# rsokolovskii/fl_scaling_sc_ldpc

Hardware: AMD Instinct MI355X
Metric: MC codeword trials/sec, (4,8) SC-LDPC L=50 N=1000 eps=0.48 full BP (higher is better)
Workload: dtype u32

## Files before the change

### fl_scaling_sc_ldpc_amd/csrc/full_bp_small.hip

```cpp
#include "common.h"
#include "kernel_util.h"
#include "table_rows.h"
#include <algorithm>
#include <cstdlib>
#include <type_traits>

namespace {

using namespace scldpc_dev;

enum { SC_NE = 0, SC_REM, SC_N0, SC_N1, SC_OVF, SC_Q, SC_N = 8 };
enum { LV_VALID = 2, LV_EXTRA0 = 3, LV_PUSH = 6, LV_DROP = 9, LV_REM = 12, LV_OVF = 15, LV_N = 18 };

struct SmArgs {
    int L, V, C, n, nk, cn_lim, nw, ncw;
    uint32_t magic_v, magic_c;
    int ntrials;
    int kswitch;
    int max_it;
    int rows_cap;
    int32_t *rows;
    int off_U, off_q0, off_q1, off_pos, off_scal, off_fb, total, qcap;
    const uint16_t *vn_adj16;
    const uint16_t *cn_adj16;
    const uint32_t *chan;
    int32_t *counters;
    uint32_t *erased_out;
    int ncaps;
    int caps[SCLDPC_MAX_CAPS];
};


template <int BLOCK, bool LEVEL, bool PERSIST, bool SOCK, bool TRAJ = false, bool CAPS = false, bool WIDE = false, int DV = 4, int DC = 8,
          int OCC = 0>
__global__ __launch_bounds__(BLOCK, OCC ? OCC : WIDE ? 4 : PERSIST ? 8 : 7) __attribute__((amdgpu_num_sgpr(96))) void full_bp_small_kernel(const SmArgs a)
{
    static_assert(!WIDE || (BLOCK == 1024 && LEVEL && SOCK && !PERSIST), "the wide form: LEVEL [+ TRAJ | CAPS], socket table");
    static_assert(!(TRAJ && CAPS), "the checkpoints have no rows form");
    static_assert((DV == 4 && DC == 8) || (SOCK && !PERSIST), "other degree pairs: the socket table, no PERSIST");
    static_assert(DC <= 15 && DC % 2 == 0 && DV < DC, "a CN's count of erased neighbours is a nibble; CN rows are read as 32-bit words");
    using QT = std::conditional_t<WIDE, uint32_t, uint16_t>;
    constexpr int kWaves = BLOCK / 64;
    extern __shared__ uint32_t lds[];
    uint32_t *cnt = lds;
    uint32_t *U = lds + a.off_U;
    QT *q[2] = {reinterpret_cast<QT *>(lds + a.off_q0), reinterpret_cast<QT *>(lds + a.off_q1)};
    int *pos_cnt = reinterpret_cast<int *>(lds + a.off_pos);
    int *pos_ss = pos_cnt + a.L;
    int *scal = reinterpret_cast<int *>(lds + a.off_scal);

    const int tid = threadIdx.x, lane = tid & 63, wave = tid >> 6;
    auto decode_trial = [&](const int trial) {
    STAMP_DECL
    const int n = a.n, nk = a.nk, cn_lim = a.cn_lim, nw = a.nw, V = a.V, C = a.C, L = a.L, qcap = a.qcap;
    const auto *vrow = reinterpret_cast<const typename VnUnit<DV>::type *>(a.vn_adj16) + (size_t)trial * n * VnUnit<DV>::per_row;
    const auto *crow = reinterpret_cast<const typename CnUnit<DC>::type *>(a.cn_adj16) + (size_t)trial * nk * CnUnit<DC>::per_row;
    auto vn_row = [&](int j) { if constexpr (DV == 4) return load_row(vrow, j); else return load_row<DV>(vrow, j); };
    auto cn_row = [&](int c) { if constexpr (DC == 8) return load_row(crow, c); else return load_row<DC>(crow, c); };
    const uint32_t *ch = a.chan + (size_t)trial * nw;

    for (int c = tid; c < a.ncw; c += BLOCK) cnt[c] = 0;
    int ne_local = 0;
    for (int w = tid; w < nw; w += BLOCK) {
        const uint32_t x = chan_tail(ch[w], w, nw, n);
        U[w] = x;
        ne_local += __popc(x);
    }
    if (tid < LV_N) scal[tid] = 0;
    for (int i = tid; i < 2 * L; i += BLOCK) pos_cnt[i] = 0;
    __syncthreads();
    ne_local = wave_sum(ne_local);
    if (lane == 0 && ne_local) atomicAdd(&scal[SC_NE], ne_local);

    constexpr int NB = 8;
    for (int j0 = tid; j0 < n; j0 += NB * BLOCK) {
        Row<DV> r[NB];
        bool er[NB];
#pragma unroll
        for (int u = 0; u < NB; u++) {
            const int j = j0 + u * BLOCK;
            er[u] = false;
            if (j < n) { r[u] = vn_row(j); er[u] = (U[j >> 5] >> (j & 31)) & 1u; }
        }
#pragma unroll
        for (int u = 0; u < NB; u++) {
            const int j = j0 + u * BLOCK;
            if (er[u]) {
                const int base = (int)__umulhi((uint32_t)j, a.magic_v) * C;
                int cc[DV];
#pragma unroll
                for (int i = 0; i < DV; i++) cc[i] = base + i * C + (int)r[u][i];
#pragma unroll
                for (int i = 0; i < DV; i++) atomicAdd(&cnt[cc[i] >> 3], 1u << ((cc[i] & 7) * 4));
            }
        }
    }
    __syncthreads();
    STAMP(0);
    const int nch = scal[SC_NE];

    int removed = 0, drops = 0;
    auto step = [&](int c, uint32_t (&out)[DV]) {
#pragma unroll
        for (int i = 0; i < DV; i++) out[i] = 0;
        const Row<DC> s = cn_row(c);
        uint32_t jk[DC];
        bool none[DC];
#pragma unroll
        for (int k = 0; k < DC; k++) { jk[k] = s[k]; none[k] = jk[k] == 0xFFFFu; }
        if constexpr (SOCK) {
            const int vbase = (int)__umulhi((uint32_t)c, a.magic_c) * V;
#pragma unroll
            for (int k = 0; k < DC; k++) jk[k] = (uint32_t)(vbase - (int)(jk[k] % DV) * V) + (jk[k] / DV);
        }
        uint32_t wd[DC];
#pragma unroll
        for (int k = 0; k < DC; k++) wd[k] = U[none[k] ? 0u : jk[k] >> 5];
        int j = -1;
#pragma unroll
        for (int k = 0; k < DC; k++)
            if (!none[k] && ((wd[k] >> (jk[k] & 31u)) & 1u)) j = (int)jk[k];
        if (j < 0) return;
        const Row<DV> r = vn_row(j);
        const uint32_t bit = 1u << (j & 31);
        if (!(atomicAnd(&U[j >> 5], ~bit) & bit)) return;
        removed++;
        const int base = (int)__umulhi((uint32_t)j, a.magic_v) * C;
        int cc[DV];
#pragma unroll
        for (int i = 0; i < DV; i++) cc[i] = base + i * C + (int)r[i];
        uint32_t o[DV];
#pragma unroll
        for (int i = 0; i < DV; i++) o[i] = atomicSub(&cnt[cc[i] >> 3], 1u << ((cc[i] & 7) * 4));
#pragma unroll
        for (int i = 0; i < DV; i++) {
            const uint32_t old = (o[i] >> ((cc[i] & 7) * 4)) & 15u;
            if (old == 2u && cc[i] < cn_lim) out[i] = (uint32_t)cc[i] + 1u;
            if constexpr (LEVEL) drops += (old == 1u && cc[i] < cn_lim);
        }
    };
    auto ones_of = [&](int w) {
        const uint32_t y = cnt[w] ^ 0x11111111u;
        uint32_t z = ~(((y & 0x77777777u) + 0x77777777u) | y) & 0x88888888u;
        if (w * 8 + 8 > cn_lim) {
            const int keep = cn_lim - w * 8;
            z = keep <= 0 ? 0u : (z & ((1u << (4 * keep)) - 1u));
        }
        return z;
    };
    auto append = [&](const uint32_t (&out)[DV], int *push, QT *qn, bool &overflow) {
        int mine = 0;
#pragma unroll
        for (int i = 0; i < DV; i++) mine += out[i] != 0u;
        const int incl = (int)wave_inclusive_scan((uint32_t)mine);
        const int tot = __builtin_amdgcn_readlane(incl, 63);
        if (tot) {
            int base = 0;
            if (lane == 0) base = atomicAdd(push, tot);
            int idx = __builtin_amdgcn_readfirstlane(base) + incl - mine;
#pragma unroll
            for (int i = 0; i < DV; i++)
                if (out[i]) { if (idx < qcap) qn[idx] = (QT)(out[i] - 1u); else overflow = true; idx++; }
        }
    };

    int rounds = 0, ne = 0, status = 0, be = 0, ee = 0, bee = 0;
    auto residual = [&]() {
    if (ne > 0) {
        for (int w = tid; w < nw; w += BLOCK) {
            uint32_t x = U[w];
            int p0 = (int)__umulhi((uint32_t)(w * 32), a.magic_v);
            int room = (p0 + 1) * V - w * 32;
            while (x) {
                const uint32_t lo = room >= 32 ? x : (x & ((1u << room) - 1u));
                if (lo) atomicAdd(&pos_cnt[p0], __popc(lo));
                x = room >= 32 ? 0u : (x >> room);
                p0++;
                room = V;
            }
        }
        __syncthreads();
        int q0 = 0;
        for (;;) {
            while (q0 < L && pos_cnt[q0] == 0) q0++;
            if (q0 >= L) break;
            for (int t = tid; t < V; t += BLOCK) {
                const int j = q0 * V + t;
                if (!((U[j >> 5] >> (j & 31)) & 1u)) continue;
                const Row<DV> r = vn_row(j);
                const int base = q0 * C;
                int cc[DV];
#pragma unroll
                for (int i = 0; i < DV; i++) cc[i] = base + i * C + (int)r[i];
                bool pair = true;
#pragma unroll
                for (int i = 0; i < DV; i++) pair = pair && ((cnt[cc[i] >> 3] >> ((cc[i] & 7) * 4)) & 15u) == 2u;
                if (!pair) continue;
                int partner = -1;
                for (int i = 0; i < DV && pair; i++) {
                    const Row<DC> s = cn_row(cc[i]);
                    int other = -1;
                    for (int k = 0; k < DC; k++) {
                        const uint32_t jk = s[k];
                        if (jk == 0xFFFFu) continue;
                        const int j2 = SOCK ? (q0 + i - (int)(jk % DV)) * V + (int)(jk / DV) : (int)jk;
                        if (j2 != j && ((U[j2 >> 5] >> (j2 & 31)) & 1u)) other = j2;
                    }
                    if (other < 0 || (i > 0 && other != partner)) pair = false;
                    partner = other;
                }
                if (pair && (int)__umulhi((uint32_t)partner, a.magic_v) == q0) atomicAdd(&pos_ss[q0], 1);
            }
            __syncthreads();
            const int e = pos_cnt[q0] - pos_ss[q0];
            if (e > 0) { ee = e; bee = 1; break; }
            q0++;
        }
        for (int pos = 0; pos < L; pos++) be += pos_cnt[pos] > 0;
    }
    };
    auto put = [&](int32_t *o, int ne, int be, int ee, int bee, int rounds, int status) {
        o[SCLDPC_C_NUM_ERASURES] = ne;
        o[SCLDPC_C_NUM_BLOCKS_ERR] = be;
        o[SCLDPC_C_NUM_ERASURES_EXP] = ee;
        o[SCLDPC_C_NUM_BLOCKS_ERR_EXP] = bee;
        o[SCLDPC_C_NUM_ERASURES_P1] = 0;
        o[SCLDPC_C_ITERATIONS] = rounds;
        o[SCLDPC_C_STATUS] = status;
        o[SCLDPC_C_CHANNEL_ERASURES] = nch;
    };
    auto cap_counters = [&](int k) { return a.counters + ((size_t)k * a.ntrials + trial) * SCLDPC_NCOUNTERS; };

    int ci = 0;
    if constexpr (LEVEL) {
        uint8_t *fb = reinterpret_cast<uint8_t *>(lds + a.off_fb);
        int prec = n, iter = 0, ncur = 0, nfront = 0, first_word = 0;
        if constexpr (TRAJ) {
            int extra = 0;
            const int head = (DV - 1) * C, tail0 = L * C;
            for (int i = tid; i < 2 * head; i += BLOCK) {
                const int c = i < head ? i : tail0 + (i - head);
                if (c >= cn_lim || c >= nk) continue;
                const Row<DC> s = cn_row(c);
                int deg = 0;
#pragma unroll
                for (int k = 0; k < DC; k++) deg += s[k] != 0xFFFFu;
                extra += deg == 1 && ((cnt[c >> 3] >> ((c & 7) * 4)) & 15u) == 0u;
            }
            extra = wave_sum(extra);
            if (lane == 0 && extra) atomicAdd(&scal[LV_EXTRA0], extra);
        }
        bool scan = true;
        ne = nch;
        for (;;) {
            const int g = iter % 3, gn = (iter + 1) % 3;
            QT *qc = q[iter & 1], *qn = q[(iter + 1) & 1];
            if (tid == 0) { scal[LV_PUSH + gn] = 0; scal[LV_DROP + gn] = 0; scal[LV_REM + gn] = 0; scal[LV_OVF + gn] = 0; }
// ... 593 lines not shown
```

### fl_scaling_sc_ldpc_amd/csrc/sampler_common.h

```cpp
#pragma once
#include "common.h"
#include "kernel_util.h"
#include <algorithm>
#include <cstdlib>

namespace scldpc {

constexpr int kSamplerThreads = 1024;
constexpr int kSamplerWaves = kSamplerThreads / 64;
constexpr int kMaxDoped = 32;
constexpr int kWorkCap = 1024;

}

namespace scldpc_dev {

__device__ __forceinline__ uint32_t channel_erased(uint32_t draw, uint32_t thresh) { return (uint32_t)((draw >> 1) < thresh); }
__device__ __forceinline__ uint32_t channel_tail(uint32_t word, int j0, int n)
{
    if (j0 + 32 > n) word &= (1u << (n - j0)) - 1u;
    return word;
}
__device__ __forceinline__ uint32_t channel_undope(uint32_t word, int j0, int pos, int vns_pos)
{
    const int lo = max(pos * vns_pos, j0) - j0, hi = min((pos + 1) * vns_pos, j0 + 32) - j0;
    if (lo < hi) word &= ~(((hi - lo) == 32 ? 0xFFFFFFFFu : ((1u << (hi - lo)) - 1u)) << lo);
    return word;
}

__device__ __forceinline__ uint32_t nib_sum(uint32_t x)
{
    const uint32_t v = (x & 0x0F0Fu) + ((x >> 4) & 0x0F0Fu);
    return (v + (v >> 8)) & 0xFFu;
}

template <int ROWS>
__device__ __forceinline__ void load_hist_words(const uint32_t *hist, int tid, uint32_t (&x)[ROWS])
{
    if constexpr (ROWS % 4 == 0) {
#pragma unroll
        for (int r = 0; r < ROWS / 4; r++) {
            const uint4 q = reinterpret_cast<const uint4 *>(hist)[tid * (ROWS / 4) + r];
            x[4 * r] = q.x; x[4 * r + 1] = q.y; x[4 * r + 2] = q.z; x[4 * r + 3] = q.w;
        }
    } else if constexpr (ROWS == 2) { const uint2 q = reinterpret_cast<const uint2 *>(hist)[tid]; x[0] = q.x; x[1] = q.y; }
    else { static_assert(ROWS == 1, "ROWS is 1, 2 or a multiple of 4"); x[0] = hist[tid]; }
}

template <int ROWS>
__device__ __forceinline__ void store_hist_words(uint32_t *hist, int tid, const uint32_t (&x)[ROWS])
{
    if constexpr (ROWS % 4 == 0) {
#pragma unroll
        for (int r = 0; r < ROWS / 4; r++)
            reinterpret_cast<uint4 *>(hist)[tid * (ROWS / 4) + r] = make_uint4(x[4 * r], x[4 * r + 1], x[4 * r + 2], x[4 * r + 3]);
    } else if constexpr (ROWS == 2) reinterpret_cast<uint2 *>(hist)[tid] = make_uint2(x[0], x[1]);
    else hist[tid] = x[0];
}

template <int ROWS>
__device__ __forceinline__ void clear_hist_words(uint32_t *hist, int tid)
{
    uint32_t z[ROWS];
#pragma unroll
    for (int r = 0; r < ROWS; r++) z[r] = 0;
    store_hist_words<ROWS>(hist, tid, z);
}

template <int ROWS, bool INCL>
__device__ __forceinline__ bool scan_hist(uint32_t *hist, uint32_t *wsum, int tid, int lane, int wave, int S)
{
    constexpr int kWaves = scldpc::kSamplerWaves;
    bool ranked = true;
    if constexpr (INCL) {
        uint32_t x[ROWS], t20[ROWS], tot20 = 0;
        load_hist_words<ROWS>(hist, tid, x);
#pragma unroll
        for (int r = 0; r < ROWS; r++) {
            x[r] *= 0x111110u;
            t20[r] = x[r] & 0xF00000u;
            tot20 += t20[r];
        }
        const uint32_t tot = tot20 >> 20, inc = wave_inclusive_scan(tot);
        if (lane == 63) wsum[wave] = inc;
        __syncthreads();
        uint32_t winc = lane < kWaves ? wsum[lane] : 0u;
        const uint32_t wt = winc;
        winc += (uint32_t)__builtin_amdgcn_update_dpp(0, (int)winc, 0x111, 0xF, 0xF, false);
        winc += (uint32_t)__builtin_amdgcn_update_dpp(0, (int)winc, 0x112, 0xF, 0xF, false);
        winc += (uint32_t)__builtin_amdgcn_update_dpp(0, (int)winc, 0x114, 0xF, 0xF, false);
        winc += (uint32_t)__builtin_amdgcn_update_dpp(0, (int)winc, 0x118, 0xF, 0xF, false);
        ranked = __builtin_amdgcn_readlane((int)winc, kWaves - 1) == S;
        uint32_t pre20 = (inc - tot + (uint32_t)__builtin_amdgcn_readlane((int)(winc - wt), wave)) << 20;
#pragma unroll
        for (int r = 0; r < ROWS; r++) {
            x[r] = (x[r] & 0xFFFF0u) | pre20;
            pre20 += t20[r];
        }
        store_hist_words<ROWS>(hist, tid, x);
    } else {
        uint32_t x[ROWS], v[ROWS], tot = 0;
        load_hist_words<ROWS>(hist, tid, x);
#pragma unroll
        for (int r = 0; r < ROWS; r++) v[r] = 0;
        if constexpr (ROWS % 2 == 0) {
#pragma unroll
            for (int r = 0; r < ROWS; r += 2) {
                const uint32_t y = x[r] | (x[r + 1] << 16);
                const uint32_t sb = (y & 0x0F0F0F0Fu) + ((y >> 4) & 0x0F0F0F0Fu);
                v[r] = (sb & 0xFFu) + ((sb >> 8) & 0xFFu);
                v[r + 1] = ((sb >> 16) & 0xFFu) + (sb >> 24);
                tot += v[r] + v[r + 1];
            }
        } else {
            static_assert(ROWS == 1 || ROWS % 2 == 0, "ROWS is 1, 2, 4 or 8");
            v[0] = nib_sum(x[0]);
            tot = v[0];
        }
        const uint32_t inc = wave_inclusive_scan(tot);
        if (lane == 63) wsum[wave] = inc;
        __syncthreads();
        const uint32_t wt = lane < kWaves ? wsum[lane] : 0u;
        const uint32_t winc = wave_inclusive_scan(wt);
        uint32_t pre = inc - tot + (uint32_t)__builtin_amdgcn_readlane((int)(winc - wt), wave);
#pragma unroll
        for (int r = 0; r < ROWS; r++) { x[r] |= pre << 16; pre += v[r]; }
        store_hist_words<ROWS>(hist, tid, x);
    }
    __syncthreads();
    if constexpr (!INCL) ranked = wsum[kWaves + 1] == 0u;
    return ranked;
}

template <int KSHIFT, int E, class Live>
__device__ __forceinline__ void bucket_ranges_excl(const uint32_t *hist, const uint32_t (&key)[E], Live &&live,
                                                   uint32_t (&g0a)[E], uint32_t (&g1a)[E])
{
    uint32_t h[E];
#pragma unroll
    for (int e = 0; e < E; e++) h[e] = hist[live(e) ? (key[e] >> KSHIFT) >> 2 : 0u];
#pragma unroll
    for (int e = 0; e < E; e++) {
        const uint32_t k4 = ((key[e] >> KSHIFT) & 3u) * 4u, x = h[e];
        const uint32_t below = x & ((1u << k4) - 1u);
        g0a[e] = (x >> 16) + (below & 0xFu) + ((below >> 4) & 0xFu) + ((below >> 8) & 0xFu);
        g1a[e] = g0a[e] + ((x >> k4) & 0xFu);
    }
}

template <int LG, bool STAGE, class Entry, class CnOf>
__device__ __forceinline__ void resolve_worklist(int nwork, int tid, const uint32_t *wl, const uint32_t *gpk, uint16_t *stage,
                                                 uint16_t *fix, Entry &&entry, CnOf &&cn_of)
{
    for (int w = tid; w < nwork; w += scldpc::kSamplerThreads) {
        const uint32_t ea = wl[2 * w], pk = wl[2 * w + 1];
        uint32_t r = ea & 0xFFFFu;
#pragma unroll 1
        for (uint32_t m = ea & 0xFFFFu; m < (ea >> 16); m++) r += gpk[m] < pk;
        const uint32_t sck = pk & ((1u << LG) - 1u);
        if constexpr (STAGE) stage[r] = entry(sck);
        fix[sck] = (uint16_t)cn_of(r);
    }
}

}

namespace scldpc {

inline uint32_t erasure_threshold(double eps)
{
    const double x = eps * 2147483647.0;
    double c = (double)(uint64_t)x;
    if (c < x) c += 1.0;
    return (uint32_t)c;
}

inline int check_sample_call(const char *who, const scldpc_code_params *p, bool bad_buffers, int32_t ntrials, double eps,
                             int32_t ndoped, const int32_t *doped_positions, int *a_ndoped, int (&a_doped)[kMaxDoped])
{
    if (bad_buffers)
        return set_error(SCLDPC_ERR_BAD_ARG, "%s: null buffer or negative ntrials", who);
    if (ndoped < 0 || ndoped > kMaxDoped || (ndoped > 0 && !doped_positions))
        return set_error(SCLDPC_ERR_BAD_ARG, "%s: 0 <= ndoped <= %d", who, kMaxDoped);
    if (!(eps >= 0.0 && eps <= 1.0))
        return set_error(SCLDPC_ERR_BAD_ARG, "%s: eps=%g outside [0,1]", who, eps);
    if (ntrials <= 0) return SCLDPC_OK;
    *a_ndoped = ndoped;
    for (int d = 0; d < ndoped; d++) {
        if (doped_positions[d] < 0 || doped_positions[d] >= p->L)
            return set_error(SCLDPC_ERR_BAD_ARG, "doped position %d outside [0,%d)", doped_positions[d], p->L);
        a_doped[d] = doped_positions[d];
    }
    return SCLDPC_OK;
}

template <class Args>
inline int v2_lds_layout(const char *who, int S, int hist_bufs, bool by_nb, bool stage, Args *a, int *lg, size_t *bytes)
{
    *lg = 10;
    while ((1 << *lg) < S) ++*lg;
    a->nb = 1 << *lg;
    const int s_lay = by_nb ? a->nb : S;
    int off = (hist_bufs * a->nb + 3) & ~3;
    a->off_gpk = off;   off += (s_lay + 3) & ~3;
    a->off_fix = off;   off += (s_lay / 2 + 3) & ~3;
    a->off_stage = off; off += stage ? (s_lay / 2 + 3) & ~3 : 0;
    a->off_wsum = off;  off += 32 + 2 * kWorkCap;
    *bytes = 4u * (size_t)off;
    *bytes = std::min(*bytes + debug_lds_pad("SAMPLER"), std::max(*bytes, (size_t)kMaxLdsBytes));
    if (*bytes > (size_t)kMaxLdsBytes)
        return set_error(SCLDPC_ERR_TOO_LARGE, "%s: %zu bytes of LDS per trial", who, *bytes);
    a->force_exact = -1;
    if (const char *v = getenv("SCLDPC_DEBUG_SAMPLER_EXACT_POS")) a->force_exact = atoi(v);
    return SCLDPC_OK;
}

constexpr int kWideHistWords = 8192;
constexpr int kWidePartCap = 12288;
constexpr int kWideMaxSockets = kWideHistWords + kWidePartCap;

template <class Args>
inline int v2_wide_lds_layout(const char *who, int S, Args *a, size_t *bytes)
{
    int off = kWideHistWords;
    a->off_gpk = off;   off += kWidePartCap;
    a->off_stage = off; off += kWidePartCap / 2;
    a->off_fix = off;   off += (S / 2 + 3) & ~3;
    a->off_wsum = off;  off += 64 + 2 * kWorkCap;
    *bytes = 4u * (size_t)off;
    *bytes = std::min(*bytes + debug_lds_pad("SAMPLER"), std::max(*bytes, (size_t)kMaxLdsBytes));
    if (S > kWideMaxSockets || *bytes > (size_t)kMaxLdsBytes)
        return set_error(SCLDPC_ERR_TOO_LARGE, "%s: %zu bytes of LDS per trial", who, *bytes);
    a->force_exact = -1;
    if (const char *v = getenv("SCLDPC_DEBUG_SAMPLER_EXACT_POS")) a->force_exact = atoi(v);
    a->part_cap = kWidePartCap;
    if (const char *v = getenv("SCLDPC_DEBUG_SAMPLER_PART_CAP")) a->part_cap = std::min(kWidePartCap, std::max(0, atoi(v)));
    return SCLDPC_OK;
}

}
```

### fl_scaling_sc_ldpc_amd/csrc/sampler_v2.hip

```cpp
#include "sampler_common.h"
#include "philox.h"

namespace {

using scldpc_dev::channel_erased;
using scldpc_dev::channel_tail;
using scldpc_dev::channel_undope;
using scldpc_dev::clear_hist_words;
using scldpc_dev::load_hist_words;
using scldpc_dev::store_hist_words;
using scldpc_dev::philox4x32_10;
using scldpc_dev::philox_prefix;
using scldpc_dev::philox_tail;
using scldpc_dev::philox_uniform;
using scldpc_dev::PhiloxPrefix;
using scldpc_dev::PhiloxUniform;
using scldpc_dev::wave_inclusive_scan;

constexpr int kThreads = scldpc::kSamplerThreads;
constexpr int kWaves = kThreads / 64;
using scldpc::kMaxDoped;
using scldpc::kWorkCap;

__device__ __forceinline__ uint32_t lds_add_rtn(uint32_t *p, uint32_t v)
{
    const uint32_t addr = (uint32_t)(uintptr_t)(__attribute__((address_space(3))) uint32_t *)p;
    uint32_t old;
    asm volatile("ds_add_rtn_u32 %0, %1, %2\n\ts_waitcnt lgkmcnt(0)" : "=v"(old) : "v"(addr), "v"(v) : "memory");
    return old;
}

struct S2Args {
    int L, cns_pos, vns_pos, n, S, D, nb, nw;
    int ntrials;
    int force_exact;
    int ndoped;
    int doped[kMaxDoped];
    uint32_t seed_lo, seed_hi;
    unsigned long long trial0;
    uint32_t thresh;
    int off_gpk, off_fix, off_stage, off_wsum;
    uint16_t *vn_adj16;
    uint16_t *cn_adj16;
    uint32_t *chan;
};

template <int ROWS, int CNMODE>
struct V2Layout {
    static constexpr int nb = ROWS * kThreads;
    static constexpr int off_gpk = nb, off_fix = off_gpk + nb, off_stage = off_fix + nb / 2;
    static constexpr int off_wsum = off_stage + (CNMODE != 0 ? nb / 2 : 0);
};

template <int KMAX, int ROWS, int CNMODE, bool PERSIST = false>
__global__ __launch_bounds__(kThreads, KMAX == 1 ? 8 : 4) __attribute__((amdgpu_num_sgpr(72))) void sample_philox_v2_kernel(const S2Args a)
{
    constexpr int DV = 4, DC_SHIFT = 3, E = 4 * KMAX;
    constexpr int LG = ROWS == 1 ? 10 : ROWS == 2 ? 11 : ROWS == 4 ? 12 : 13;
    constexpr int KSHIFT = 32 - LG - 2;
    constexpr bool INCL = KMAX == 1;
    static_assert(ROWS * kThreads == (1 << LG) && (INCL ? ROWS <= 4 : ROWS == 8), "ROWS is 1, 2, 4 (KMAX 1) or 8 (KMAX 2)");
    extern __shared__ uint32_t lds[];
    using Lay = V2Layout<ROWS, CNMODE>;
    const int off_gpk = INCL ? Lay::off_gpk : a.off_gpk, off_fix = INCL ? Lay::off_fix : a.off_fix;
    const int off_stage = INCL ? Lay::off_stage : a.off_stage, off_wsum = INCL ? Lay::off_wsum : a.off_wsum;
    uint32_t *hist = lds;
    uint32_t *gpk = lds + off_gpk;
    uint16_t *fix = reinterpret_cast<uint16_t *>(lds + off_fix);
    uint16_t *stage = reinterpret_cast<uint16_t *>(lds + off_stage);
    uint32_t *wsum = lds + off_wsum;
    uint32_t *wl = wsum + 32;

    const int tid = threadIdx.x, lane = tid & 63, wave = __builtin_amdgcn_readfirstlane(tid >> 6);
    const int S = a.S, nb = INCL ? ROWS * kThreads : a.nb;
    const int ncalls = S >> 2;
    bool own[KMAX];
#pragma unroll
    for (int k = 0; k < KMAX; k++) own[k] = tid + k * kThreads < ncalls;
    auto sock = [&](int e) { return (uint32_t)((tid + (e >> 2) * kThreads) * 4 + (e & 3)); };
    auto stage_entry = [&](int p, uint32_t sck) -> uint16_t {
        const int u = (int)(sck & 3u), t = (int)(sck >> 2);
        if ((unsigned)(p - u) >= (unsigned)a.L) return (uint16_t)0xFFFFu;
        return CNMODE == 1 ? (uint16_t)((p - u) * a.vns_pos + t) : (uint16_t)sck;
    };

    STAMP_DECL
    for (int b = tid; b < nb; b += kThreads) hist[b] = 0;
    if (tid == 0) { wsum[kWaves] = 0; wsum[kWaves + 1] = 0; }
    __syncthreads();
    auto sample_trial = [&](const int tr) {
    const unsigned long long trial = a.trial0 + (unsigned long long)tr;
    const uint32_t t_lo = (uint32_t)trial, t_hi = (uint32_t)(trial >> 32);
    uint32_t rowP[KMAX], rowQ[KMAX], rowR[KMAX];
#pragma unroll
    for (int k = 0; k < KMAX; k++) rowP[k] = rowQ[k] = rowR[k] = 0;
    PhiloxPrefix pre[KMAX];
#pragma unroll
    for (int k = 0; k < KMAX; k++) pre[k] = philox_prefix((uint32_t)(tid + k * kThreads), t_lo, t_hi, a.seed_lo, a.seed_hi);
    uint32_t nxt[E];
    {
        const PhiloxUniform un = philox_uniform(0u, t_lo, a.seed_lo, a.seed_hi);
#pragma unroll
        for (int k = 0; k < KMAX; k++) {
            uint32_t r[4] = {0, 0, 0, 0};
            if (own[k]) philox_tail(pre[k], un, a.seed_lo, a.seed_hi, r);
#pragma unroll
            for (int u = 0; u < 4; u++) nxt[4 * k + u] = r[u];
        }
    }
    for (int p = 0; p < a.D; p++) {
        STAMP(0);
        uint32_t key[E], slot[E], crowded = 0;
        auto word_of = [](uint32_t k) { return (k >> KSHIFT) & ~3u; };
        auto nib_of = [](uint32_t k) { return (k >> (KSHIFT - 2)) & 12u; };
#pragma unroll
        for (int e = 0; e < E; e++) {
            key[e] = nxt[e];
            const uint32_t sh = nib_of(key[e]);
            uint32_t *w = reinterpret_cast<uint32_t *>(reinterpret_cast<char *>(hist) + word_of(key[e]));
            slot[e] = (atomicAdd(w, (own[e >> 2] ? 1u : 0u) << sh) >> sh) & 0xFu;
            if constexpr (!INCL) crowded = max(crowded, slot[e]);
        }
        if (!INCL && crowded >= 15u) wsum[kWaves + 1] = 1u;
        __syncthreads();
        STAMP(1);

        const bool ranked = scldpc_dev::scan_hist<ROWS, INCL>(hist, wsum, tid, lane, wave, S);
        STAMP(2);

        if (ranked) {
            uint32_t rk[E], g0a[E], g1a[E];
            bool st[E], sx[E];
            if constexpr (INCL) {
                uint32_t h[E];
#pragma unroll
                for (int e = 0; e < E; e++) h[e] = *reinterpret_cast<const uint32_t *>(reinterpret_cast<const char *>(hist) + word_of(key[e]));
#pragma unroll
                for (int e = 0; e < E; e++) {
                    const uint32_t t = h[e] >> nib_of(key[e]), pre = h[e] >> 20;
                    g0a[e] = pre + (t & 0xFu);
                    g1a[e] = pre + ((t >> 4) & 0xFu);
                    rk[e] = g0a[e] + slot[e];
                    sx[e] = ((g0a[e] ^ (g1a[e] - 1u)) >> DC_SHIFT) != 0u;
                    st[e] = own[e >> 2] && sx[e];
                }
            } else {
                scldpc_dev::bucket_ranges_excl<KSHIFT>(hist, key, [&](int e) { return own[e >> 2]; }, g0a, g1a);
#pragma unroll
                for (int e = 0; e < E; e++) {
                    rk[e] = g0a[e] + slot[e];
                    st[e] = own[e >> 2] && ((g1a[e] - 1u) >> DC_SHIFT) != (g0a[e] >> DC_SHIFT);
                }
            }
            if constexpr (INCL) {
                const unsigned long long ownv = __builtin_amdgcn_ballot_w64(own[0]);
                unsigned long long vote[E];
                int total = 0;
#pragma unroll
                for (int e = 0; e < E; e++) { vote[e] = __builtin_amdgcn_ballot_w64(sx[e]) & ownv; total += __builtin_popcountll(vote[e]); }
                if (total != 0) {
                    uint32_t ln, got = 0;
                    asm volatile("v_and_b32 %0, 63, %1" : "=v"(ln) : "v"(tid));
                    if (ln == 0u) got = lds_add_rtn(&wsum[kWaves], (uint32_t)total);
                    int base = __builtin_amdgcn_readfirstlane((int)got);
                    if (base + total <= kWorkCap) {
                        static_assert((Lay::off_wsum + 32) % 2 == 0, "the worklist starts on a word pair");
                        uint2 *wl2 = reinterpret_cast<uint2 *>(lds);
                        base += (Lay::off_wsum + 32) / 2;
#pragma unroll
                        for (int e = 0; e < E; e++) {
                            if (st[e]) {
                                const uint32_t w = __builtin_amdgcn_mbcnt_hi((uint32_t)(vote[e] >> 32),
                                                                             __builtin_amdgcn_mbcnt_lo((uint32_t)vote[e], (uint32_t)base));
                                const uint32_t pk = (key[e] << LG) | sock(e);
                                gpk[rk[e]] = pk;
                                uint32_t *ent = reinterpret_cast<uint32_t *>(wl2 + w);
                                ent[0] = g0a[e] | (g1a[e] << 16);
                                ent[1] = pk;
                            }
                            base += __builtin_popcountll(vote[e]);
                        }
                    }
                }
            } else {
                uint32_t smask = 0;
#pragma unroll
                for (int e = 0; e < E; e++) smask |= (st[e] ? 1u : 0u) << e;
                while (smask) {
                    const uint32_t e = (uint32_t)__ffs((int)smask) - 1u;
                    smask &= smask - 1u;
                    uint32_t ky = key[0], r0 = rk[0], g0 = g0a[0], g1 = g1a[0];
#pragma unroll
                    for (int f = 1; f < E; f++)
                        if (e == (uint32_t)f) { ky = key[f]; r0 = rk[f]; g0 = g0a[f]; g1 = g1a[f]; }
                    const uint32_t pk = (ky << LG) | (uint32_t)((tid + (int)(e >> 2) * kThreads) * 4 + (int)(e & 3u));
                    gpk[r0] = pk;
                    const int w = atomicAdd(reinterpret_cast<int *>(&wsum[kWaves]), 1);
                    if (w < kWorkCap) { wl[2 * w] = g0 | (g1 << 16); wl[2 * w + 1] = pk; }
                }
            }
#pragma unroll
            for (int k = 0; k < KMAX; k++) {
                if (!own[k]) continue;
                uint2 v;
                v.x = (rk[4 * k] >> DC_SHIFT) | ((rk[4 * k + 1] >> DC_SHIFT) << 16);
                v.y = (rk[4 * k + 2] >> DC_SHIFT) | ((rk[4 * k + 3] >> DC_SHIFT) << 16);
                reinterpret_cast<uint2 *>(fix)[tid + k * kThreads] = v;
            }
            if constexpr (CNMODE != 0) {
#pragma unroll
                for (int k = 0; k < KMAX; k++) {
                    if (!own[k]) continue;
#pragma unroll
                    for (int u = 0; u < 4; u++) stage[rk[4 * k + u]] = stage_entry(p, sock(4 * k + u));
                }
            }
        }
        __syncthreads();
        STAMP(3);

        {
            clear_hist_words<ROWS>(hist, tid);
            int nwork = (int)wsum[kWaves];
            const bool exact = !ranked || nwork > kWorkCap || a.force_exact == p || a.force_exact == -2;
            if (exact) {
                asm volatile("; ledger: cold");
                nwork = 0;
#pragma unroll
                for (int e = 0; e < E; e++) if (own[e >> 2]) gpk[sock(e)] = key[e];
                __syncthreads();
                uint32_t xr[E];
#pragma unroll
                for (int e = 0; e < E; e++) xr[e] = 0;
                for (int s2 = 0; s2 < S; s2++) {
                    const uint32_t k2 = gpk[s2];
#pragma unroll
                    for (int e = 0; e < E; e++) xr[e] += (k2 < key[e]) || (k2 == key[e] && (uint32_t)s2 < sock(e));
                }
#pragma unroll
                for (int k = 0; k < KMAX; k++) {
                    if (!own[k]) continue;
                    uint2 v;
                    v.x = (xr[4 * k] >> DC_SHIFT) | ((xr[4 * k + 1] >> DC_SHIFT) << 16);
                    v.y = (xr[4 * k + 2] >> DC_SHIFT) | ((xr[4 * k + 3] >> DC_SHIFT) << 16);
                    reinterpret_cast<uint2 *>(fix)[tid + k * kThreads] = v;
                    if constexpr (CNMODE != 0) {
#pragma unroll
                        for (int u = 0; u < 4; u++) stage[xr[4 * k + u]] = stage_entry(p, sock(4 * k + u));
                    }
                }
            }
            scldpc_dev::resolve_worklist<LG, CNMODE != 0>(nwork, tid, wl, gpk, stage, fix, [&](uint32_t sck) { return stage_entry(p, sck); },
                                                          [](uint32_t r) { return r >> DC_SHIFT; });
        }
        if (p + 1 < a.D) {
            uint32_t k_lo = a.seed_lo, k_hi = a.seed_hi;
            uint32_t tl = t_lo;
            asm volatile("" : "+s"(k_lo), "+s"(k_hi), "+s"(tl));
            const PhiloxUniform un = philox_uniform((uint32_t)(p + 1), tl, k_lo, k_hi);
#pragma unroll
            for (int k = 0; k < KMAX; k++) {
                uint32_t r[4] = {0, 0, 0, 0};
                if (own[k]) philox_tail(pre[k], un, k_lo, k_hi, r);
#pragma unroll
                for (int u = 0; u < 4; u++) nxt[4 * k + u] = r[u];
            }
        }
        __syncthreads();
        if (tid == 0) { wsum[kWaves] = 0; wsum[kWaves + 1] = 0; }
        STAMP(4);

        const int qpos = p - (DV - 1);
#pragma unroll
        for (int k = 0; k < KMAX; k++) {
            uint2 c = make_uint2(0u, 0u);
            if (own[k]) c = reinterpret_cast<const uint2 *>(fix)[tid + k * kThreads];
            if (qpos >= 0 && own[k]) {
                const size_t j = (size_t)tr * a.n + (size_t)((uint32_t)qpos * (uint32_t)a.vns_pos + (uint32_t)(tid + k * kThreads));
                uint2 v;
                v.x = rowP[k];
                v.y = (rowR[k] >> 16) | (c.y & 0xFFFF0000u);
                reinterpret_cast<uint2 *>(a.vn_adj16)[j] = v;
            }
            rowP[k] = rowQ[k];
            rowQ[k] = (rowR[k] & 0xFFFFu) | (c.x & 0xFFFF0000u);
            rowR[k] = (c.x & 0xFFFFu) | (c.y << 16);
        }
        if constexpr (CNMODE != 0) {
            uint2 *dst = reinterpret_cast<uint2 *>(a.cn_adj16) + ((size_t)tr * a.D + p) * (size_t)(S >> 2);
            const uint2 *src = reinterpret_cast<const uint2 *>(stage);
            for (int w = tid; w < (S >> 2); w += kThreads) dst[w] = src[w];
        }
        STAMP(5);
    }

    uint32_t *chan = a.chan + (size_t)tr * a.nw;
    const PhiloxUniform chun = philox_uniform(0x80000000u, t_lo, a.seed_lo, a.seed_hi);
    for (int w = tid; w < a.nw; w += kThreads) {
        uint32_t word = 0;
#pragma unroll
        for (int c = 0; c < 8; c++) {
            uint32_t r[4];
            philox_tail(philox_prefix((uint32_t)(w * 8 + c), t_lo, t_hi, a.seed_lo, a.seed_hi), chun, a.seed_lo, a.seed_hi, r);
#pragma unroll
            for (int u = 0; u < 4; u++) word |= channel_erased(r[u], a.thresh) << (c * 4 + u);
        }
        const int j0 = w * 32;
        word = channel_tail(word, j0, a.n);
        for (int d = 0; d < a.ndoped; d++) word = channel_undope(word, j0, a.doped[d], a.vns_pos);
        chan[w] = word;
    }
    STAMP(6);
    };
    if constexpr (PERSIST) {
        for (int tr = blockIdx.x; tr < a.ntrials; tr += gridDim.x) {
            sample_trial(tr);
            __syncthreads();
        }
    } else {
        sample_trial((int)blockIdx.x);
    }
    STAMP_FLUSH();
}


__device__ __forceinline__ uint32_t wl_entry_vn(const S2Args &a, int p, uint32_t sck)
{
    return (uint32_t)((p - (int)(sck & 3u)) * a.vns_pos + (int)(sck >> 2));
}

template <int LG, int CNMODE>
__global__ __launch_bounds__(kThreads, 8) __attribute__((amdgpu_num_sgpr(72))) void sample_philox_v3_kernel(const S2Args a)
{
    constexpr int DV = 4, DC_SHIFT = 3, E = 4;
    constexpr int NB = 1 << LG, ROWS = NB / kThreads;
    constexpr int KSHIFT = 32 - LG - 2;
    constexpr uint32_t LOWMASK = (1u << KSHIFT) - 1u;
    constexpr int SBITS = LG;
    static_assert(ROWS == 1 || ROWS == 2 || ROWS == 4, "one Philox call per thread: at most 4096 sockets per position");
    extern __shared__ uint32_t lds[];
    uint32_t *hist0 = lds;
    uint32_t *gpk = lds + a.off_gpk;
    uint16_t *fix = reinterpret_cast<uint16_t *>(lds + a.off_fix);
    uint16_t *stage = reinterpret_cast<uint16_t *>(lds + a.off_stage);
    uint32_t *wsum = lds + a.off_wsum;
    uint32_t *wl = wsum + 32;

    const int tid = threadIdx.x, lane = tid & 63, wave = tid >> 6;
    const int S = a.S;
    const bool own = tid < (S >> 2);
    const unsigned long long trial = a.trial0 + blockIdx.x;
    const uint32_t t_lo = (uint32_t)trial, t_hi = (uint32_t)(trial >> 32);
    const int tr = blockIdx.x;

    STAMP_DECL
    for (int b = tid; b < 2 * NB; b += kThreads) hist0[b] = 0;
    if (tid < 32) wsum[tid] = 0;
    __syncthreads();

    uint32_t rowP = 0, rowQ = 0, rowR = 0;
    uint32_t key[E] = {0, 0, 0, 0}, slot[E] = {0, 0, 0, 0};
    uint32_t ent0 = CNMODE == 1 ? (uint32_t)tid : (uint32_t)(4 * tid);
    uint32_t vV = (uint32_t)a.vns_pos;
    asm volatile("" : "+v"(vV));

    for (int p = 0; p <= a.D; p++) {
        uint32_t *hc = hist0 + (p & 1) * NB, *hp = hist0 + ((p & 1) ^ 1) * NB;
        const bool live = p < a.D;
        STAMP(0);
        if (p > 0) {
            int nwork = (int)wsum[16];
            const bool exact = wsum[18 + ((p - 1) & 1)] != 0u || nwork > kWorkCap || a.force_exact == p - 1 || a.force_exact == -2;
            if (exact) {
                uint32_t k2[4] = {0, 0, 0, 0};
                uint32_t f_lo = a.seed_lo, f_hi = a.seed_hi;
                asm volatile("" : "+s"(f_lo), "+s"(f_hi));
                if (own) philox4x32_10((uint32_t)tid, (uint32_t)(p - 1), t_lo, t_hi, f_lo, f_hi, k2);
                if (own) { gpk[4 * tid] = k2[0]; gpk[4 * tid + 1] = k2[1]; gpk[4 * tid + 2] = k2[2]; gpk[4 * tid + 3] = k2[3]; }
                __syncthreads();
                uint32_t xr[4] = {0, 0, 0, 0};
                for (int s2 = 0; s2 < S; s2++) {
                    const uint32_t kk = gpk[s2];
#pragma unroll
                    for (int u = 0; u < 4; u++) xr[u] += (kk < k2[u]) || (kk == k2[u] && s2 < 4 * tid + u);
                }
                if (own) {
                    uint2 v;
                    v.x = (xr[0] >> DC_SHIFT) | ((xr[1] >> DC_SHIFT) << 16);
                    v.y = (xr[2] >> DC_SHIFT) | ((xr[3] >> DC_SHIFT) << 16);
                    reinterpret_cast<uint2 *>(fix)[tid] = v;
                    if constexpr (CNMODE != 0) {
#pragma unroll
                        for (int u = 0; u < 4; u++) {
                            const int pu = p - 1 - u;
                            stage[xr[u]] = (unsigned)pu < (unsigned)a.L ? (uint16_t)(CNMODE == 1 ? pu * a.vns_pos + tid : 4 * tid + u) : (uint16_t)0xFFFFu;
                        }
                    }
                }
                nwork = 0;
            }
            for (int w = tid; w < nwork; w += kThreads) {
                const uint32_t ea = wl[2 * w], pk = wl[2 * w + 1];
                const uint32_t g0 = ea & 0xFFFFu, cnt = (ea >> 16) & 0xFu, sl = (ea >> 20) & 0xFu;
                uint32_t r = g0;
                for (uint32_t m = 0; m < cnt; m++)
                    if (m != sl) r += gpk[g0 + m] < pk;
                const uint32_t sck = pk & ((1u << SBITS) - 1u);
                if constexpr (CNMODE != 0) stage[r] = (uint16_t)(ea >> 24 ? 0xFFFFu : (CNMODE == 1 ? wl_entry_vn(a, p - 1, sck) : sck));
                fix[sck] = (uint16_t)(r >> DC_SHIFT);
            }
            {
                clear_hist_words<ROWS>(hp, tid);
            }
        }
        STAMP(1);
        if (live) {
            {
                uint32_t k_lo = a.seed_lo, k_hi = a.seed_hi;
                asm volatile("" : "+s"(k_lo), "+s"(k_hi));
                uint32_t r[4] = {0, 0, 0, 0};
                if (own) philox4x32_10((uint32_t)tid, (uint32_t)p, t_lo, t_hi, k_lo, k_hi, r);
#pragma unroll
                for (int u = 0; u < 4; u++) key[u] = r[u];
            }
            uint32_t crowded = 0;
#pragma unroll
            for (int e = 0; e < E; e++) {
                const uint32_t boff = (key[e] >> KSHIFT) & ~3u, sh = (key[e] >> (KSHIFT - 2)) & 12u;
                const uint32_t old = atomicAdd(reinterpret_cast<uint32_t *>(reinterpret_cast<char *>(hc) + boff), (own ? 16u : 0u) << sh);
                slot[e] = (old >> (sh + 4u)) & 0xFu;
                crowded |= slot[e] + 1u;
            }
            if (crowded & 16u) wsum[18 + (p & 1)] = 1u;
        }
        STAMP(2);
        __syncthreads();
        STAMP(3);
        if (tid == 0) { wsum[16] = 0; wsum[18 + ((p & 1) ^ 1)] = 0; }
        if (live) {
            uint32_t x[ROWS], tot = 0, over = 0;
            load_hist_words<ROWS>(hc, tid, x);
            uint32_t v[ROWS];
#pragma unroll
            for (int r = 0; r < ROWS; r++) {
                const uint32_t y = x[r] * 0x1111u;
// ... 21 lines not shown
                vv.x = rowP;
                vv.y = (rowR >> 16) | (c.y & 0xFFFF0000u);
                reinterpret_cast<uint2 *>(a.vn_adj16)[j] = vv;
            }
            rowP = rowQ;
            rowQ = (rowR & 0xFFFFu) | (c.x & 0xFFFF0000u);
            rowR = (c.x & 0xFFFFu) | (c.y << 16);
            if constexpr (CNMODE != 0) {
                uint2 *dst = reinterpret_cast<uint2 *>(a.cn_adj16) + ((size_t)tr * a.D + pp) * (size_t)(S >> 2);
                const uint2 *src = reinterpret_cast<const uint2 *>(stage);
                if (own) dst[tid] = src[tid];
            }
        }
        STAMP(4);
        __syncthreads();
        STAMP(5);
        if (live && wsum[18 + (p & 1)] == 0u) {
            const uint32_t wt = lane < kWaves ? wsum[lane] : 0u;
            uint32_t wi = wt;
            wi += (uint32_t)__builtin_amdgcn_update_dpp(0, (int)wi, 0x111, 0xF, 0xF, false);
            wi += (uint32_t)__builtin_amdgcn_update_dpp(0, (int)wi, 0x112, 0xF, 0xF, false);
            wi += (uint32_t)__builtin_amdgcn_update_dpp(0, (int)wi, 0x114, 0xF, 0xF, false);
            wi += (uint32_t)__builtin_amdgcn_update_dpp(0, (int)wi, 0x118, 0xF, 0xF, false);
            const uint32_t wex = wi - wt;
            uint32_t h[E], wb[E], rk[E], g0a[E], cnta[E];
#pragma unroll
            for (int e = 0; e < E; e++) h[e] = *reinterpret_cast<const uint32_t *>(reinterpret_cast<const char *>(hc) + ((key[e] >> KSHIFT) & ~3u));
#pragma unroll
            for (int e = 0; e < E; e++) wb[e] = (uint32_t)__builtin_amdgcn_ds_bpermute((int)((key[e] >> 26) & 0x3Cu), (int)wex);
            bool st[E];
            bool anyst = false;
#pragma unroll
            for (int e = 0; e < E; e++) {
                const uint32_t t1 = h[e] >> ((key[e] >> (KSHIFT - 2)) & 12u);
                const uint32_t excl = t1 & 15u, incl = (t1 >> 4) & 15u;
                g0a[e] = (h[e] >> 20) + wb[e] + excl;
                cnta[e] = incl - excl;
                rk[e] = g0a[e] + slot[e];
                st[e] = own && ((g0a[e] ^ (g0a[e] + cnta[e] - 1u)) >> DC_SHIFT) != 0u;
                anyst = anyst || st[e];
            }
            if (own) {
                uint2 vv;
                vv.x = (rk[0] >> DC_SHIFT) | ((rk[1] >> DC_SHIFT) << 16);
                vv.y = (rk[2] >> DC_SHIFT) | ((rk[3] >> DC_SHIFT) << 16);
                reinterpret_cast<uint2 *>(fix)[tid] = vv;
            }
            const bool edge = p < DV - 1 || p >= a.L;
            if constexpr (CNMODE != 0) {
                if (own) {
                    uint32_t ent[E];
                    ent[0] = ent0;
#pragma unroll
                    for (int u = 1; u < 4; u++) ent[u] = CNMODE == 1 ? ent[u - 1] - vV : ent[u - 1] + 1u;
                    if (!edge) {
#pragma unroll
                        for (int u = 0; u < 4; u++) stage[rk[u]] = (uint16_t)ent[u];
                    } else {
#pragma unroll
                        for (int u = 0; u < 4; u++) stage[rk[u]] = (unsigned)(p - u) < (unsigned)a.L ? (uint16_t)ent[u] : (uint16_t)0xFFFFu;
                    }
                }
            }
            if (__builtin_amdgcn_ballot_w64(anyst)) {
                unsigned long long vote[E];
                int total = 0;
#pragma unroll
                for (int e = 0; e < E; e++) { vote[e] = __builtin_amdgcn_ballot_w64(st[e]); total += __builtin_popcountll(vote[e]); }
                int base = 0;
                if (lane == 0) base = atomicAdd(reinterpret_cast<int *>(&wsum[16]), total);
                base = __builtin_amdgcn_readfirstlane(base);
#pragma unroll
                for (int e = 0; e < E; e++) {
                    if (st[e]) {
                        const int w = base + (int)__builtin_amdgcn_mbcnt_hi((uint32_t)(vote[e] >> 32), __builtin_amdgcn_mbcnt_lo((uint32_t)vote[e], 0u));
                        const uint32_t pk = ((key[e] & LOWMASK) << SBITS) | (uint32_t)(4 * tid + e);
                        gpk[g0a[e] + slot[e]] = pk;
                        const uint32_t none = CNMODE != 0 && edge && !((unsigned)(p - e) < (unsigned)a.L) ? 1u : 0u;
                        if (w < kWorkCap) { wl[2 * w] = g0a[e] | (cnta[e] << 16) | (slot[e] << 20) | (none << 24); wl[2 * w + 1] = pk; }
                    }
                    base += __builtin_popcountll(vote[e]);
                }
            }
        }
        if constexpr (CNMODE == 1) ent0 += vV;
        STAMP(6);
        __syncthreads();
        STAMP(7);
    }

    uint32_t *chan = a.chan + (size_t)tr * a.nw;
    for (int w = tid; w < a.nw; w += kThreads) {
        uint32_t word = 0;
        uint32_t c_lo = a.seed_lo, c_hi = a.seed_hi;
        asm volatile("" : "+s"(c_lo), "+s"(c_hi));
#pragma unroll
        for (int c = 0; c < 8; c++) {
            uint32_t r[4];
            philox4x32_10((uint32_t)(w * 8 + c), 0x80000000u, t_lo, t_hi, c_lo, c_hi, r);
#pragma unroll
            for (int u = 0; u < 4; u++) word |= channel_erased(r[u], a.thresh) << (c * 4 + u);
        }
        const int j0 = w * 32;
        word = channel_tail(word, j0, a.n);
        for (int d = 0; d < a.ndoped; d++) word = channel_undope(word, j0, a.doped[d], a.vns_pos);
        chan[w] = word;
    }
    STAMP(8);
    STAMP_FLUSH();
}

int launch_v2(const char *who, int cnmode, const scldpc_code_params *p, uint64_t seed, uint64_t trial0, int32_t ntrials,
              double eps, int32_t ndoped, const int32_t *doped_positions, uint16_t *d_vn_adj16, uint16_t *d_table,
              uint32_t *d_chan_bits, void *stream)
{
    S2Args a{};
    if (int rc = scldpc::check_sample_call(who, p, ntrials < 0 || (ntrials > 0 && (!d_vn_adj16 || !d_chan_bits)), ntrials, eps,
                                           ndoped, doped_positions, &a.ndoped, a.doped)) return rc;
    if (ntrials == 0) return SCLDPC_OK;
    if (!d_table) cnmode = 0;

    a.L = p->L; a.cns_pos = p->cns_pos; a.vns_pos = p->vns_pos;
    a.n = scldpc::n_of(p); a.S = p->cns_pos * p->dc; a.D = p->L + p->dv - 1; a.nw = scldpc::nw_of(p);
    a.seed_lo = (uint32_t)seed; a.seed_hi = (uint32_t)(seed >> 32);
    a.trial0 = trial0;
    a.thresh = scldpc::erasure_threshold(eps);
    const char *gen_env = getenv("SCLDPC_SAMPLER_GEN");
    const bool one_call = a.S <= 4 * kThreads;
    const bool v3 = one_call && gen_env && atoi(gen_env) == 3;
    int lg;
    size_t lds_bytes;
    if (int rc = scldpc::v2_lds_layout(who, a.S, v3 ? 2 : 1, one_call && !v3, cnmode != 0, &a, &lg, &lds_bytes)) return rc;
    a.vn_adj16 = d_vn_adj16; a.cn_adj16 = d_table; a.chan = d_chan_bits;
    a.ntrials = ntrials;

    using Kern = void (*)(const S2Args);
    static const Kern table[4][3] = {
        {sample_philox_v2_kernel<1, 1, 0>, sample_philox_v2_kernel<1, 1, 1>, sample_philox_v2_kernel<1, 1, 2>},
        {sample_philox_v2_kernel<1, 2, 0>, sample_philox_v2_kernel<1, 2, 1>, sample_philox_v2_kernel<1, 2, 2>},
        {sample_philox_v2_kernel<1, 4, 0>, sample_philox_v2_kernel<1, 4, 1>, sample_philox_v2_kernel<1, 4, 2>},
        {sample_philox_v2_kernel<2, 8, 0>, sample_philox_v2_kernel<2, 8, 1>, sample_philox_v2_kernel<2, 8, 2>},
    };
    const int rows = a.nb / kThreads;
    static const Kern table3[3][3] = {
        {sample_philox_v3_kernel<10, 0>, sample_philox_v3_kernel<10, 1>, sample_philox_v3_kernel<10, 2>},
        {sample_philox_v3_kernel<11, 0>, sample_philox_v3_kernel<11, 1>, sample_philox_v3_kernel<11, 2>},
        {sample_philox_v3_kernel<12, 0>, sample_philox_v3_kernel<12, 1>, sample_philox_v3_kernel<12, 2>},
    };
    const int grid = v3 ? ntrials : scldpc::debug_grid("SAMPLER", ntrials);
    Kern kern = v3 ? table3[lg - 10][cnmode] : table[rows == 1 ? 0 : rows == 2 ? 1 : rows == 4 ? 2 : 3][cnmode];
    if (grid < ntrials && rows == 4 && cnmode == 1) kern = sample_philox_v2_kernel<1, 4, 1, true>;
    else if (grid < ntrials) return scldpc::set_error(SCLDPC_ERR_BAD_ARG, "SCLDPC_DEBUG_GRID_SAMPLER: only the <1,4,1> kernel has a persistent form");
    if (int rc_ = scldpc::allow_max_lds(reinterpret_cast<const void *>(kern))) return rc_;
    hipLaunchKernelGGL(kern, dim3(grid), dim3(kThreads), lds_bytes, static_cast<hipStream_t>(stream), a);
    SCLDPC_HIP_CHECK(hipGetLastError());
    return SCLDPC_OK;
}

bool v2_shape(const scldpc_code_params *p)
{
    if (scldpc::check_params(p)) return false;
    const int S = p->cns_pos * p->dc;
    return p->dv == 4 && p->dc == 8 && (S & 3) == 0 && S <= 8192 && p->vns_pos * p->dv == S;
}

}

extern "C" int scldpc_sample_philox_cn16_supported(const scldpc_code_params *p)
{
    return v2_shape(p) && scldpc::n_of(p) < 65535;
}

extern "C" int scldpc_sample_philox_sock16_supported(const scldpc_code_params *p)
{
    return v2_shape(p);
}

extern "C" int scldpc_sample_philox_device_cn16(const scldpc_code_params *p, uint64_t seed, uint64_t trial0,
                                                int32_t ntrials, double eps, int32_t ndoped,
                                                const int32_t *doped_positions, uint16_t *d_vn_adj16,
                                                uint16_t *d_cn_adj16, uint32_t *d_chan_bits, void *stream)
{
    const char *who = "scldpc_sample_philox_device_cn16";
    if (int rc = scldpc::check_params(p)) return rc;
    if (!scldpc_sample_philox_cn16_supported(p))
        return scldpc::set_error(SCLDPC_ERR_TOO_LARGE, "%s: takes dv = 4, dc = 8, at most 8192 sockets per position and "
                                 "fewer than 65535 VNs (got dv=%d dc=%d cns_pos=%d n=%d)", who, p->dv, p->dc, p->cns_pos,
                                 scldpc::n_of(p));
    return launch_v2(who, 1, p, seed, trial0, ntrials, eps, ndoped, doped_positions, d_vn_adj16, d_cn_adj16, d_chan_bits,
                     stream);
}

extern "C" int scldpc_sample_philox_device_sock16(const scldpc_code_params *p, uint64_t seed, uint64_t trial0,
                                                  int32_t ntrials, double eps, int32_t ndoped,
                                                  const int32_t *doped_positions, uint16_t *d_vn_adj16,
                                                  uint16_t *d_cn_sock16, uint32_t *d_chan_bits, void *stream)
{
    const char *who = "scldpc_sample_philox_device_sock16";
    if (int rc = scldpc::check_params(p)) return rc;
    if (!scldpc_sample_philox_sock16_supported(p))
        return scldpc::set_error(SCLDPC_ERR_TOO_LARGE, "%s: takes dv = 4, dc = 8 and at most 8192 sockets per position "
                                 "(got dv=%d dc=%d cns_pos=%d)", who, p->dv, p->dc, p->cns_pos);
    return launch_v2(who, 2, p, seed, trial0, ntrials, eps, ndoped, doped_positions, d_vn_adj16, d_cn_sock16, d_chan_bits,
                     stream);
}
```

Baseline: 1.249 million.

## Skip zero-count checks in BP step and address sampler LDS by absolute offsets

In the full-BP peeling step, a check node whose packed erasure count is zero now returns early, before its row is loaded and the U words are read. In the sampler's inclusive path, LDS atomics, loads and stores use raw address-space-3 byte offsets, with a v_add doubling trick for 16-bit indexing. For CNMODE 1 the stage entries are computed incrementally rather than recomputed. A host check rejects kernels with static LDS, because the hardcoded offsets assume none.

```diff
diff --git a/fl_scaling_sc_ldpc_amd/csrc/full_bp_small.hip b/fl_scaling_sc_ldpc_amd/csrc/full_bp_small.hip
--- a/fl_scaling_sc_ldpc_amd/csrc/full_bp_small.hip
+++ b/fl_scaling_sc_ldpc_amd/csrc/full_bp_small.hip
@@ -103,6 +103,9 @@
     auto step = [&](int c, uint32_t (&out)[DV]) {
 #pragma unroll
         for (int i = 0; i < DV; i++) out[i] = 0;
+        if constexpr (!LEVEL) {
+            if (((cnt[c >> 3] >> ((c & 7) * 4)) & 15u) == 0u) return;
+        }
         const Row<DC> s = cn_row(c);
         uint32_t jk[DC];
         bool none[DC];
diff --git a/fl_scaling_sc_ldpc_amd/csrc/sampler_common.h b/fl_scaling_sc_ldpc_amd/csrc/sampler_common.h
--- a/fl_scaling_sc_ldpc_amd/csrc/sampler_common.h
+++ b/fl_scaling_sc_ldpc_amd/csrc/sampler_common.h
@@ -26,6 +26,18 @@
     const int lo = max(pos * vns_pos, j0) - j0, hi = min((pos + 1) * vns_pos, j0 + 32) - j0;
     if (lo < hi) word &= ~(((hi - lo) == 32 ? 0xFFFFFFFFu : ((1u << (hi - lo)) - 1u)) << lo);
     return word;
+}
+
+template <class T>
+__device__ __forceinline__ __attribute__((address_space(3))) T *lds_at(uint32_t byte)
+{
+    return (__attribute__((address_space(3))) T *)(uintptr_t)byte;
+}
+__device__ __forceinline__ uint32_t twice(uint32_t x)
+{
+    uint32_t y;
+    asm("v_add_u32 %0, %1, %1" : "=v"(y) : "v"(x));
+    return y;
 }
 
 __device__ __forceinline__ uint32_t nib_sum(uint32_t x)
@@ -148,7 +160,7 @@
     }
 }
 
-template <int LG, bool STAGE, class Entry, class CnOf>
+template <int LG, bool STAGE, int STAGE_BYTE = -1, int FIX_BYTE = -1, class Entry, class CnOf>
 __device__ __forceinline__ void resolve_worklist(int nwork, int tid, const uint32_t *wl, const uint32_t *gpk, uint16_t *stage,
                                                  uint16_t *fix, Entry &&entry, CnOf &&cn_of)
 {
@@ -158,8 +170,13 @@
 #pragma unroll 1
         for (uint32_t m = ea & 0xFFFFu; m < (ea >> 16); m++) r += gpk[m] < pk;
         const uint32_t sck = pk & ((1u << LG) - 1u);
-        if constexpr (STAGE) stage[r] = entry(sck);
-        fix[sck] = (uint16_t)cn_of(r);
+        if constexpr (FIX_BYTE >= 0) {
+            if constexpr (STAGE) *lds_at<uint16_t>(twice(r) + (uint32_t)STAGE_BYTE) = entry(sck);
+            *lds_at<uint16_t>(twice(sck) + (uint32_t)FIX_BYTE) = (uint16_t)cn_of(r);
+        } else {
+            if constexpr (STAGE) stage[r] = entry(sck);
+            fix[sck] = (uint16_t)cn_of(r);
+        }
     }
 }
 
diff --git a/fl_scaling_sc_ldpc_amd/csrc/sampler_v2.hip b/fl_scaling_sc_ldpc_amd/csrc/sampler_v2.hip
--- a/fl_scaling_sc_ldpc_amd/csrc/sampler_v2.hip
+++ b/fl_scaling_sc_ldpc_amd/csrc/sampler_v2.hip
@@ -7,8 +7,10 @@
 using scldpc_dev::channel_tail;
 using scldpc_dev::channel_undope;
 using scldpc_dev::clear_hist_words;
+using scldpc_dev::lds_at;
 using scldpc_dev::load_hist_words;
 using scldpc_dev::store_hist_words;
+using scldpc_dev::twice;
 using scldpc_dev::philox4x32_10;
 using scldpc_dev::philox_prefix;
 using scldpc_dev::philox_tail;
@@ -108,6 +110,8 @@
             for (int u = 0; u < 4; u++) nxt[4 * k + u] = r[u];
         }
     }
+    [[maybe_unused]] uint32_t ent0 = (uint32_t)tid, vV = (uint32_t)a.vns_pos;
+    if constexpr (CNMODE == 1 && INCL) asm volatile("" : "+v"(vV));
     for (int p = 0; p < a.D; p++) {
         STAMP(0);
         uint32_t key[E], slot[E], crowded = 0;
@@ -117,9 +121,14 @@
         for (int e = 0; e < E; e++) {
             key[e] = nxt[e];
             const uint32_t sh = nib_of(key[e]);
-            uint32_t *w = reinterpret_cast<uint32_t *>(reinterpret_cast<char *>(hist) + word_of(key[e]));
-            slot[e] = (atomicAdd(w, (own[e >> 2] ? 1u : 0u) << sh) >> sh) & 0xFu;
-            if constexpr (!INCL) crowded = max(crowded, slot[e]);
+            if constexpr (INCL) {
+                slot[e] = (__hip_atomic_fetch_add(lds_at<uint32_t>(word_of(key[e])), (own[e >> 2] ? 1u : 0u) << sh, __ATOMIC_RELAXED,
+                                                  __HIP_MEMORY_SCOPE_WORKGROUP) >> sh) & 0xFu;
+            } else {
+                uint32_t *w = reinterpret_cast<uint32_t *>(reinterpret_cast<char *>(hist) + word_of(key[e]));
+                slot[e] = (atomicAdd(w, (own[e >> 2] ? 1u : 0u) << sh) >> sh) & 0xFu;
+                crowded = max(crowded, slot[e]);
+            }
         }
         if (!INCL && crowded >= 15u) wsum[kWaves + 1] = 1u;
         __syncthreads();
@@ -134,7 +143,7 @@
             if constexpr (INCL) {
                 uint32_t h[E];
 #pragma unroll
-                for (int e = 0; e < E; e++) h[e] = *reinterpret_cast<const uint32_t *>(reinterpret_cast<const char *>(hist) + word_of(key[e]));
+                for (int e = 0; e < E; e++) h[e] = *lds_at<const uint32_t>(word_of(key[e]));
 #pragma unroll
                 for (int e = 0; e < E; e++) {
                     const uint32_t t = h[e] >> nib_of(key[e]), pre = h[e] >> 20;
@@ -207,7 +216,24 @@
                 v.y = (rk[4 * k + 2] >> DC_SHIFT) | ((rk[4 * k + 3] >> DC_SHIFT) << 16);
                 reinterpret_cast<uint2 *>(fix)[tid + k * kThreads] = v;
             }
-            if constexpr (CNMODE != 0) {
+            if constexpr (CNMODE != 0 && INCL) {
+                if (own[0]) {
+                    uint32_t ent[4], at[4];
+                    ent[0] = CNMODE == 1 ? ent0 : sock(0);
+#pragma unroll
+                    for (int u = 1; u < 4; u++) ent[u] = CNMODE == 1 ? ent[u - 1] - vV : sock(u);
+#pragma unroll
+                    for (int u = 0; u < 4; u++) {
+                        at[u] = twice(rk[u]);
+                        *lds_at<uint16_t>(at[u] + 4u * Lay::off_stage) = (uint16_t)ent[u];
+                    }
+                    if (p < DV - 1 || p >= a.L) {
+#pragma unroll
+                        for (int u = 0; u < 4; u++)
+                            if ((unsigned)(p - u) >= (unsigned)a.L) *lds_at<uint16_t>(at[u] + 4u * Lay::off_stage) = (uint16_t)0xFFFFu;
+                    }
+                }
+            } else if constexpr (CNMODE != 0) {
 #pragma unroll
                 for (int k = 0; k < KMAX; k++) {
                     if (!own[k]) continue;
@@ -250,8 +276,8 @@
                     }
                 }
             }
-            scldpc_dev::resolve_worklist<LG, CNMODE != 0>(nwork, tid, wl, gpk, stage, fix, [&](uint32_t sck) { return stage_entry(p, sck); },
-                                                          [](uint32_t r) { return r >> DC_SHIFT; });
+            scldpc_dev::resolve_worklist<LG, CNMODE != 0, INCL ? 4 * Lay::off_stage : -1, INCL ? 4 * Lay::off_fix : -1>(
+                nwork, tid, wl, gpk, stage, fix, [&](uint32_t sck) { return stage_entry(p, sck); }, [](uint32_t r) { return r >> DC_SHIFT; });
         }
         if (p + 1 < a.D) {
             uint32_t k_lo = a.seed_lo, k_hi = a.seed_hi;
@@ -291,6 +317,7 @@
             const uint2 *src = reinterpret_cast<const uint2 *>(stage);
             for (int w = tid; w < (S >> 2); w += kThreads) dst[w] = src[w];
         }
+        if constexpr (CNMODE == 1 && INCL) ent0 += vV;
         STAMP(5);
     }
 
@@ -618,6 +645,13 @@
     if (grid < ntrials && rows == 4 && cnmode == 1) kern = sample_philox_v2_kernel<1, 4, 1, true>;
     else if (grid < ntrials) return scldpc::set_error(SCLDPC_ERR_BAD_ARG, "SCLDPC_DEBUG_GRID_SAMPLER: only the <1,4,1> kernel has a persistent form");
     if (int rc_ = scldpc::allow_max_lds(reinterpret_cast<const void *>(kern))) return rc_;
+    if (one_call && !v3) {
+        hipFuncAttributes fa;
+        SCLDPC_HIP_CHECK(hipFuncGetAttributes(&fa, reinterpret_cast<const void *>(kern)));
+        if (fa.sharedSizeBytes != 0)
+            return scldpc::set_error(SCLDPC_ERR_HIP, "%s: the kernel holds %zu bytes of static LDS, its addresses assume none", who,
+                                     (size_t)fa.sharedSizeBytes);
+    }
     hipLaunchKernelGGL(kern, dim3(grid), dim3(kThreads), lds_bytes, static_cast<hipStream_t>(stream), a);
     SCLDPC_HIP_CHECK(hipGetLastError());
     return SCLDPC_OK;
```

Result: no change. 1.254 million (median of 6 runs) (+0.4%).
